# liulab-dfci/TRUST4

Measured on AMD Instinct MI355X. Metric: stage-1 assembly read pairs/sec (150 bp PE), whole stage 1, higher is better.
Workload: dtype int32/u64

## Files before the change

trust4_amd/csrc/t4_api.hip:

```cpp
#include <hip/hip_runtime.h>
#include <math.h>
#include <stdarg.h>
#include <stdio.h>
#include <string.h>
#include <zlib.h>

#include <algorithm>
#include <atomic>
#include <chrono>
#include <map>
#include <mutex>
#include <string>
#include <thread>
#include <unordered_map>
#include <vector>

#ifdef __HIPCC__
#include <dlfcn.h>
#include <rccl/rccl.h>
#include <type_traits>
#include <unistd.h>
#endif
#include "../../include/trust4_hip.h"
#include "t4_kernels.h"
// ... 230 lines not shown
  }
  int r;
  if (reads > w.maxReads) {
    int n = w.maxReads > 0 ? w.maxReads : 64;
    while (n < reads) n *= 2;
    if ((r = devAlloc(c, &w.seed, 2 * (size_t)n * T4_WIDE_SEEDS))) return r;
    if ((r = devAlloc(c, &w.bounds, 2 * (size_t)n * (T4_WIDE_MAXP + 1)))) return r;
    if ((r = devAlloc(c, &w.uniqPref, 2 * (size_t)n * (w.pcap + 1)))) return r;
    if ((r = devAlloc(c, &w.sortTmp, 2 * (size_t)n * 2 * w.pcap))) return r;
    w.maxReads = n;
  }
  if (parts > w.maxPart) {
    int n = w.maxPart > 0 ? w.maxPart : wideEnv("T4_WIDE_PARTS", 1024);
    while (n < parts) n *= 2;
    const size_t n2 = 2 * (size_t)n;
    if ((r = devAlloc(c, &w.pCnt, n2))) return r;
    if ((r = devAlloc(c, &w.pRead, n2))) return r;
    if ((r = devAlloc(c, &w.pKeys, n2 * w.pcap))) return r;
    if ((r = devAlloc(c, &w.gSize, n2 * w.pcap))) return r;
    if ((r = devAlloc(c, &w.gInfo, n2 * w.pcap))) return r;
    if ((r = devAlloc(c, &w.gCount, n2 * 4))) return r;
    if ((r = devAlloc(c, &w.gOff, n2 * 2))) return r;
    if ((r = devAlloc(c, &w.pRec, n2 * w.maxOvPart * 10))) return r;
    if ((r = devAlloc(c, &w.pRecCnt, n2))) return r;
    if ((r = devAlloc(c, &w.mKeys, n2 * w.maxOvPart))) return r;
    if ((r = devAlloc(c, &w.mOrd, n2 * w.maxOvPart))) return r;
    w.maxPart = n;
  }
  if (groups > w.grpCap) {
    int n = w.grpCap > 0 ? w.grpCap : wideEnv("T4_WIDE_GROUPS", 1 << 20);
    while (n < groups) n *= 2;
    if (c->grpPoolHost) (void)hipHostFree(c->grpPoolHost);
    c->grpPoolHost = nullptr; w.grpPool = nullptr;
    HIPCHK(c, hipHostMalloc(&c->grpPoolHost, sizeof(T4Grp) * 2 * (size_t)n, hipHostMallocMapped));
    HIPCHK(c, hipHostGetDevicePointer((void **)&w.grpPool, c->grpPoolHost, 0));
    w.grpCap = n;
  }
  return T4_OK;
}
T4Wide wideHalf(const t4_ctx *c, int half) {
  T4Wide w = c->wide;
  if (!half) return w;
  const size_t R = (size_t)w.maxReads, P = (size_t)w.maxPart;
  w.seed += R * T4_WIDE_SEEDS; w.bounds += R * (T4_WIDE_MAXP + 1); w.uniqPref += R * (w.pcap + 1); w.sortTmp += R * 2 * w.pcap;
  w.pCnt += P; w.pRead += P; w.pKeys += P * w.pcap; w.gSize += P * w.pcap; w.gInfo += P * w.pcap; w.gCount += P * 4; w.gOff += P * 2;
  w.pRec += P * w.maxOvPart * 10; w.pRecCnt += P; w.mKeys += P * w.maxOvPart; w.mOrd += P * w.maxOvPart;
  w.grpPool += w.grpCap;
  return w;
}

}

extern "C" {

int t4_init(int device_ordinal, t4_ctx **out) {
  if (!out) return T4_ERR_ARG;
  *out = nullptr;
  int ndev = 0;
  if (hipGetDeviceCount(&ndev) != hipSuccess || ndev <= 0 || device_ordinal < 0 || device_ordinal >= ndev) return T4_ERR_HIP;
  if (hipSetDevice(device_ordinal) != hipSuccess) return T4_ERR_HIP;
  t4_ctx *c = new t4_ctx();
  c->device = device_ordinal;
  hipDeviceProp_t prop;
  if (hipGetDeviceProperties(&prop, device_ordinal) != hipSuccess) { delete c; return T4_ERR_HIP; }
  c->cus = prop.multiProcessorCount;
  if (hipStreamCreate(&c->stream) != hipSuccess) { delete c; return T4_ERR_HIP; }
  for (int i = 0; i < 4; ++i) if (hipEventCreate(&c->ev[i]) != hipSuccess) { delete c; return T4_ERR_HIP; }
  memset(&c->stats, 0, sizeof c->stats);
  if (hipMalloc(&c->listCounts, sizeof(int) * 16) != hipSuccess || hipMalloc(&c->hitCounter, sizeof(unsigned long long)) != hipSuccess) { delete c; return T4_ERR_HIP; }
  if (hipHostMalloc(&c->aqFlagHost, 64, hipHostMallocMapped) != hipSuccess || hipHostGetDevicePointer((void **)&c->aqFlagDev, c->aqFlagHost, 0) != hipSuccess ||
      hipMalloc(&c->aqDoneCtr, sizeof(unsigned)) != hipSuccess || hipMemset(c->aqDoneCtr, 0, sizeof(unsigned)) != hipSuccess) { delete c; return T4_ERR_HIP; }
  *c->aqFlagHost = 0;
  *out = c;
  return T4_OK;
}

void t4_destroy(t4_ctx *c) {
  if (!c) return;
  (void)hipSetDevice(c->device);
#ifdef T4_PHASE_TIMING
  if (getenv("T4_PHASE_DUMP")) {
    unsigned long long ph[T4_NPHASE];
    if (hipMemcpyFromSymbol(ph, HIP_SYMBOL(t4k::g_phaseCycles), sizeof(ph)) == hipSuccess) {
      static const char *names[32] = {"other", "seed:lookup", "expand", "sort", "stats", "runs", "bigsort", "chain", "ovsort", "score", "prefilter", "final", "annotate", "score:quick", "score:banded", "score:finish", "extend:ungapped", "after-extend", "extend:list", "extend:dp4", "extend:dp1", "extend:combine", "seed:replay", "seed:scan", "extend:launch", "-", "-", "-", "-", "-", "-", "-"};
      unsigned long long tot = 0;
      for (int i = 0; i < T4_NPHASE; ++i) tot += ph[i];
      for (int i = 0; i < T4_NPHASE; ++i) if (ph[i]) fprintf(stderr, "phase %-16s %-7s %6.2f%%  %.3e cycles\n", names[i & 31], i < 32 ? "lds" : "global", 100.0 * (double)ph[i] / (double)tot, (double)ph[i]);
    }
    static unsigned long long cls[4 * T4_NPHASE];
    if (hipMemcpyFromSymbol(cls, HIP_SYMBOL(t4k::g_phaseByOverlaps), sizeof(cls)) == hipSuccess) {
      static const char *names[32] = {"other", "seed:lookup", "expand", "sort", "stats", "runs", "bigsort", "chain", "ovsort", "score", "prefilter", "final", "annotate", "score:quick", "score:banded", "score:finish", "extend:ungapped", "after-extend", "extend:list", "extend:dp4", "extend:dp1", "extend:combine", "seed:replay", "seed:scan", "extend:launch", "-", "-", "-", "-", "-", "-", "-"};
      static const char *cname[4] = {"<5 overlaps", "5-19 overlaps", "20-64 overlaps", ">64 overlaps"};
      for (int k = 0; k < 4; ++k) {
        unsigned long long tot = 0;
        for (int i = 0; i < T4_NPHASE; ++i) tot += cls[k * T4_NPHASE + i];
        if (!tot) continue;
        fprintf(stderr, "AddRead queries with %s: %.3e cycles in the query kernel\n", cname[k], (double)tot);
        for (int i = 0; i < T4_NPHASE; ++i) if (cls[k * T4_NPHASE + i] * 200 >= tot) fprintf(stderr, "   %-16s %-7s %6.2f%%\n", names[i & 31], i < 32 ? "lds" : "global", 100.0 * (double)cls[k * T4_NPHASE + i] / (double)tot);
      }
    }
    unsigned long long dc[8];
    if (hipMemcpyFromSymbol(dc, HIP_SYMBOL(t4k::g_dbgCount), sizeof(dc)) == hipSuccess)
      fprintf(stderr, "debug counters: gap jobs %llu, banded %llu, wave-DP steps %llu, scratch fallbacks %llu; overhang DPs %llu, of which %llu leave the diagonal\n", dc[0], dc[1], dc[2], dc[3], dc[6], dc[7]);
  }
#endif
  void *ptrs[] = {c->dpRows, c->dpDir, c->gKeys, c->gPairs, c->gCand, c->gOv, c->gFin, c->gOrd, c->hitsKeys, c->lists,
                  c->listCounts, c->status, c->counts, c->hitCounter, c->result, c->aqIn, c->aqOut};
  if (c->aqInHost) (void)hipHostFree(c->aqInHost);
  if (c->aqOutHost) (void)hipHostFree(c->aqOutHost);
  if (c->aqFlagHost) (void)hipHostFree(c->aqFlagHost);
  if (c->aqDoneCtr) (void)hipFree(c->aqDoneCtr);
  if (c->aqPool) (void)hipHostFree(c->aqPool);
  if (c->candPool) (void)hipHostFree(c->candPool);
  if (c->aqRecDev) (void)hipFree(c->aqRecDev);
  if (c->aqRecRead) (void)hipFree(c->aqRecRead);
  if (c->wideInit) {
    void *wp[] = {c->wide.seed, c->wide.bounds, c->wide.pCnt, c->wide.pRead, c->wide.pKeys, c->wide.gSize, c->wide.gInfo, c->wide.gCount, c->wide.gOff, c->wide.pRec,
                  c->wide.pRecCnt, c->wide.uniqPref, c->wide.mKeys, c->wide.mOrd, c->wide.sortTmp};
    for (void *p : wp) if (p) (void)hipFree(p);
    if (c->grpPoolHost) (void)hipHostFree(c->grpPoolHost);
  }
  for (void *p : ptrs) if (p) (void)hipFree(p);
  for (int i = 0; i < 4; ++i) if (c->ev[i]) (void)hipEventDestroy(c->ev[i]);
  if (c->stream) (void)hipStreamDestroy(c->stream);
  if (c->stream2) (void)hipStreamDestroy(c->stream2);
  if (c->evIn) (void)hipEventDestroy(c->evIn);
  if (c->evG) (void)hipEventDestroy(c->evG);
  delete c;
}

int t4_sync(t4_ctx *c) {
  if (!c) return T4_ERR_ARG;
  HIPCHK(c, hipStreamSynchronize(c->stream));
  return T4_OK;
}
const char *t4_last_error(t4_ctx *c) { return c ? c->err.c_str() : "null ctx"; }
int t4_device_cus(t4_ctx *c) { return c ? c->cus : 0; }
int t4_ctx_device(t4_ctx *c) { return c ? c->device : 0; }
#ifdef T4_PHASE_TIMING
int t4_debug_phase_cycles(unsigned long long *out16) {
  unsigned long long zero[T4_NPHASE] = {0};
  if (hipMemcpyFromSymbol(out16, HIP_SYMBOL(t4k::g_phaseCycles), sizeof(zero)) != hipSuccess) return T4_ERR_HIP;
  if (hipMemcpyToSymbol(HIP_SYMBOL(t4k::g_phaseCycles), zero, sizeof(zero)) != hipSuccess) return T4_ERR_HIP;
  return T4_OK;
}
int t4_debug_counters(unsigned long long *out8) {
  unsigned long long zero[8] = {0};
  if (hipMemcpyFromSymbol(out8, HIP_SYMBOL(t4k::g_dbgCount), sizeof(zero)) != hipSuccess) return T4_ERR_HIP;
  if (hipMemcpyToSymbol(HIP_SYMBOL(t4k::g_dbgCount), zero, sizeof(zero)) != hipSuccess) return T4_ERR_HIP;
  return T4_OK;
}
#endif
int t4_debug_phase_reset(void) {
#ifdef T4_PHASE_TIMING
  unsigned long long zero[T4_NPHASE] = {0};
  if (hipMemcpyToSymbol(HIP_SYMBOL(t4k::g_phaseCycles), zero, sizeof(zero)) != hipSuccess) return T4_ERR_HIP;
#endif
  return T4_OK;
}
int t4_last_stats(t4_ctx *c, t4_stats *out) {
  if (!c || !out) return T4_ERR_ARG;
  *out = c->stats;
  return T4_OK;
}

int t4_index_create(t4_ctx *c, int k, int consider_barcode, t4_index **out) {
  if (!c || !out) return T4_ERR_ARG;
  if (k < 2 || k > 31) return fail(c, T4_ERR_ARG, "kmer_length %d outside [2,31]", k);
  t4_index *ix = new t4_index();
  ix->ctx = c; ix->k = k; ix->considerBarcode = consider_barcode ? 1 : 0;
  double kmerHitProb = pow(0.8, k);
  ix->nomatchGapLimit = int(k * (log(0.01) / log(1 - kmerHitProb))) + 1;
  *out = ix;
  return T4_OK;
// ... 2339 lines not shown
```

trust4_amd/csrc/t4_kernels.h:

```cpp
#pragma once
#include <hip/hip_runtime.h>

#include "t4_device.h"

namespace t4k {

#ifdef T4_INLINE_ALL
#define T4_NI
#else
#define T4_NI __attribute__((noinline))
#endif
#ifndef T4_OPT_JOBSORT
#define T4_OPT_JOBSORT 1
#endif
#ifndef T4_OPT_ROWWALK
#define T4_OPT_ROWWALK 1
#endif
#ifndef T4_NI_R3
#define T4_NI_R3 0
#endif
#ifdef __HIPCC__
#define T4_LDS_AS __attribute__((address_space(3)))
#else
#define T4_LDS_AS
// ... 1471 lines not shown
  if (ix.radius > 0) {
    const int wave = lane >> 6, nw = NT >> 6, wl = lane & 63;
    for (int c = wave; c < nCand; c += nw) {
      int s = CAND_START(wm.cand[c]), n = CAND_LEN(wm.cand[c]);
      if (n <= 48) continue;
      unsigned long long ks = wm.keys[s];
      if (!seqIsRef(ix, KEY_IDX(ks))) continue;
      unsigned *tmp = (unsigned *)(wm.keys + s) + n;
      for (int t = wl; t < n; t += 64) {
        unsigned long long kt = wm.keys[s + t];
        int b = KEY_B(kt), a = KEY_C(kt) - T4_C_BIAS + b;
        wm.pairs[s + t] = ((unsigned)b << 12) | (unsigned)a;
      }
      waveLdsSync();
#if T4_OPT_R2CHECK
      {
        bool unsorted = false;
        for (int t = wl + 1; t < n; t += 64) unsorted = unsorted || wm.pairs[s + t - 1] > wm.pairs[s + t];
        if (!__any(unsorted)) continue;
      }
#endif
      for (int t = wl; t < n; t += 64) {
        unsigned v = wm.pairs[s + t];
        int rank = 0;
        for (int u = 0; u < n; ++u) { unsigned x = wm.pairs[s + u]; rank += (x < v) ? 1 : 0; }
        tmp[rank] = v;
      }
      waveLdsSync();
      for (int t = wl; t < n; t += 64) wm.pairs[s + t] = tmp[t];
      waveLdsSync();
    }
  }
  __syncthreads();
  PHASE_MARK(ws, 7);
#if T4_OPT_ROWCHAIN
  chainRunsRows(ix, wm, ws, nCand, hitLenRequired);
  __syncthreads();
}
#else
  for (int c = lane; c < nCand; c += NT) {
    int s = CAND_START(wm.cand[c]), n = CAND_LEN(wm.cand[c]);
    unsigned long long ks = wm.keys[s];
    int idx = KEY_IDX(ks), plus = KEY_PLUS(ks);
    bool isRef = seqIsRef(ix, idx);
    int adjustRadius = isRef ? ix.radius : 0;
    if (!(adjustRadius > 0 && n > 48)) {
      for (int t = s; t < s + n; ++t) {
        unsigned long long kt = wm.keys[t];
        int b = KEY_B(kt), a = KEY_C(kt) - T4_C_BIAS + b;
        wm.pairs[t] = ((unsigned)b << 12) | (unsigned)a;
      }
      if (adjustRadius > 0) {
        for (int t = s + 1; t < s + n; ++t) {
          unsigned v = wm.pairs[t];
          int u = t - 1;
          while (u >= s && wm.pairs[u] > v) { wm.pairs[u + 1] = wm.pairs[u]; --u; }
          wm.pairs[u + 1] = v;
        }
      }
    }
    chainRun(ix, wm, ws, s, n, idx, plus, isRef, hitLenRequired);
  }
  __syncthreads();
}
#endif

__device__ __forceinline__ bool lowComplex(const WaveMem &wm, bool plus, int rs, int re) {
  int lo = plus ? rs : wm.segLen - 1 - re, hi = plus ? re : wm.segLen - 1 - rs;
  lo += wm.segAbs; hi += wm.segAbs;
  int cA = 0, cC = 0, cG = 0, cT = 0;
  for (int w = lo >> 4; w <= (hi >> 4); ++w) {
    const unsigned x = wm.pkRow[w];
    unsigned nb = (wm.nmRow[w >> 1] >> ((w & 1) * 16)) & 0xFFFFu;
    nb = (nb | (nb << 8)) & 0x00FF00FFu; nb = (nb | (nb << 4)) & 0x0F0F0F0Fu;
    nb = (nb | (nb << 2)) & 0x33333333u; nb = (nb | (nb << 1)) & 0x55555555u;
    unsigned v = 0x55555555u & ~nb;
    const int b0 = w << 4;
    if (lo > b0) v &= ~0u << ((lo - b0) * 2);
    if (hi < b0 + 15) v &= ~0u >> ((b0 + 15 - hi) * 2);
    const unsigned l = x & 0x55555555u, h = (x >> 1) & 0x55555555u;
    cA += __popc(~h & ~l & v); cC += __popc(~h & l & v); cG += __popc(h & ~l & v); cT += __popc(h & l & v);
  }
  const int cnt[4] = {cA, cC, cG, cT};
  int lowCnt = 0, lowTotal = 0;
  for (int i = 0; i < 4; ++i) if (cnt[i] <= 2) { ++lowCnt; lowTotal += cnt[i]; }
  if (lowTotal * 7 >= re - rs + 1) return false;
  return lowCnt >= 2;
}

__device__ bool dpAffineQuick(const char *t, int lent, const char *p, int lenp, unsigned &cnt) {
  cnt = 0;
  if (lent == 0 || lenp == 0) return true;
  if (lent != lenp) return false;
  int mm = 0;
  for (int i = 0; i < lent; ++i) { char a = t[i], b = p[i]; mm += (a == b || a == 'N' || b == 'N') ? 0 : 1; }
  if (lent > 1 && mm > 3) return false;
  cnt = CNT_MATCH * (unsigned)(lent - mm) + CNT_MIS * (unsigned)mm;
  return true;
}
__device__ bool dpPosWeightQuick(const T4PW *w, int lent, const char *p, int lenp, unsigned &cnt) {
  cnt = 0;
  if (lent == 0 || lenp == 0) return true;
  if (lent != lenp) return false;
  int mm = 0;
  for (int i = 0; i < lent; ++i) mm += baseEqualW(w[i], p[i]) ? 0 : 1;
  if (lent > 1 && !((lent - mm) * 2 - mm * 2 >= lent * 2 - 8)) return false;
  cnt = CNT_MATCH * (unsigned)(lent - mm) + CNT_MIS * (unsigned)mm;
  return true;
}

template <bool PW>
__device__ unsigned dpWave(const char *t, const T4PW *w, int lent, const char *p, int lenp, char *tbuf) {
  const int d = laneId();
  if (lent == 0 || lenp == 0) return 0u;
  if (lent == 1 && lenp == 1) {
    bool eq = PW ? baseEqualW(w[0], p[0]) : (t[0] == p[0] || t[0] == 'N' || p[0] == 'N');
    return eq ? CNT_MATCH : CNT_MIS;
  }
  if (PW && lent == lenp) {
    int mm = 0;
    for (int i = d; i < lent; i += 64) mm += baseEqualW(w[i], p[i]) ? 0 : 1;
    mm = waveSum(mm);
    if ((lent - mm) * 2 - mm * 2 >= lent * 2 - 8) return CNT_MATCH * (unsigned)(lent - mm) + CNT_MIS * (unsigned)mm;
  }
  int leftBand = 5, rightBand = 5;
  if (lent > lenp) rightBand += lent - lenp; else if (lent < lenp) leftBand += lenp - lent;
  const int W = leftBand + rightBand + 1;
  if (W > 64 || lent > T4_MAXGAP || lenp > T4_MAXGAP) return DP_FAIL;
  for (int i = d; i < lent; i += 64) tbuf[i] = PW ? (char)w[i] : t[i];
  const int negInf = (lent + 1) * (lenp + 1) * (-4);
  const int e0 = -4 + (lenp + 1) * (-4);
  const int q4 = 4 * (lenp + 1);
  int M = negInf, E = negInf, F = negInf;
  unsigned C0 = 0, C1 = 0, C2 = 0;
  {
    int j0 = d - leftBand;
    if (d < W && j0 >= 0 && j0 <= lent) {
      if (j0 == 0) { M = 0; E = 0; F = 0; }
      else if (PW) { M = -4 - 4 * j0; C0 = CNT_MATCH + CNT_INDEL * (unsigned)(j0 - 1); }
      else { M = -4 - 4 * j0; E = e0; F = -4 - j0; C0 = CNT_INDEL * (unsigned)(j0 + (j0 > q4 ? 1 : 0)); C1 = CNT_INDEL * (unsigned)(1 + j0); C2 = CNT_INDEL * (unsigned)j0; }
    }
  }
  const int lastStep = 2 * lenp + W - 1;
  for (int s = 2; s <= lastStep; ++s) {
    int lM = waveUp1(M), uM = waveDown1(M);
    unsigned lC0 = waveUp1(C0), uC0 = waveDown1(C0);
    int lF = 0, uE = 0; unsigned lC2 = 0, uC1 = 0;
    if (!PW) { lF = waveUp1(F); lC2 = waveUp1(C2); uE = waveDown1(E); uC1 = waveDown1(C1); }
    const int i2 = s - d, i = i2 >> 1, j = i - leftBand + d;
    if (d < W && (i2 & 1) == 0 && i >= 1 && i <= lenp && j >= 1 && j <= lent) {
      if (j == 1) {
        lM = -4 - 4 * i;
        if (PW) lC0 = CNT_MATCH + CNT_INDEL * (unsigned)(i - 1);
        else { lF = -4 - 4 * i; lC0 = CNT_INDEL * (unsigned)i; lC2 = CNT_INDEL * (unsigned)(1 + i); }
      } else if (d == 0) { lM = negInf; lF = negInf; lC0 = 0; lC2 = 0; }
      if (i == 1) {
        uM = -4 - 4 * j;
        if (PW) uC0 = CNT_MATCH + CNT_INDEL * (unsigned)(j - 1);
        else { uE = e0; uC0 = CNT_INDEL * (unsigned)(j + (j > q4 ? 1 : 0)); uC1 = CNT_INDEL * (unsigned)(1 + j); }
      } else if (d + 1 >= W) { uM = negInf; uE = negInf; uC0 = 0; uC1 = 0; }
      int dM; unsigned dC0;
      if (i == 1) {
        int jj = j - 1;
        dM = jj == 0 ? 0 : -4 - 4 * jj;
        dC0 = jj == 0 ? 0u : (PW ? CNT_MATCH + CNT_INDEL * (unsigned)(jj - 1) : CNT_INDEL * (unsigned)(jj + (jj > q4 ? 1 : 0)));
      } else if (j == 1) {
// ... 278 lines not shown
  int anyFast = 0;
  if (ALL && !rowsForAll) {
    for (int i = lane; i < overlapCnt; i += NT) {
      OvRec oc = wm.ov[wm.ord[i]];
      if ((oc.flags & OV_ISREF) != 0 && ix.radius > 0) anyFast = 1;
      else walkOverlap(ix, wm, ws, oc, i, true);
    }
    if (blockSum(anyFast, ws->red) == 0) return;
  }
  for (int i0 = 0; i0 < overlapCnt; i0 += nRows) {
    const int i = i0 + row;
    const bool has = i < overlapCnt;
    int chainPos = 0, chainLen = 0, ovSlot = 0;
    bool fast = false;
    if (has) {
      ovSlot = wm.ord[i];
      const OvRec &o = wm.ov[ovSlot];
      chainPos = o.chainPos; chainLen = o.chainLen;
      fast = (o.flags & OV_ISREF) != 0 && ix.radius > 0;
      if (!ALL && !fast && rl == 0) { OvRec oc = o; walkOverlap(ix, wm, ws, oc, i, true); }
    }
    const unsigned *hc = (const unsigned *)(wm.keys + chainPos);
    int jStop = 0x7FFFFFFF;
    const bool slow = ALL && has && !fast && rowsForAll;
    if (slow)
      for (int j = 1 + rl; j < chainLen; j += 16) {
        const unsigned pp = hc[j - 1], cp = hc[j];
        const int pa = PA(pp), pb = PB(pp), qa = PA(cp), qb = PB(cp);
        if (pb - pa != qb - qa || (pa + K - 1 < qa && (qb - (pb + K) > ix.nomatchGapLimit || qa - (pa + K) > ix.nomatchGapLimit))) { jStop = j; break; }
      }
    if (fast)
      for (int j = 1 + rl; j < chainLen; j += 16) {
        const unsigned pp = hc[j - 1], cp = hc[j];
        const int pa = PA(pp), pb = PB(pp), qa = PA(cp), qb = PB(cp);
        const bool gapA = pa + K - 1 < qa, gapB = pb + K - 1 < qb;
        const bool doDP = (pb - pa == qb - qa) ? gapA : (gapA && gapB);
        if (doDP && (qb - (pb + K) > ix.nomatchGapLimit || qa - (pa + K) > ix.nomatchGapLimit)) { jStop = j; break; }
      }
    for (int m = 1; m < 16; m <<= 1) { const int other = __shfl_xor(jStop, m); jStop = other < jStop ? other : jStop; }
    int matchCnt = 0, indelCnt = 0;
    if (slow)
      for (int j = 1 + rl; j < chainLen && j < jStop; j += 16) {
        if (PA(hc[j - 1]) + K - 1 < PA(hc[j])) {
          const int slot = atomicAdd(&ws->jobCount, 1);
          if (slot < wm.candCap) wm.cand[slot] = (unsigned)i | ((unsigned)j << 16); else ws->overflow = 1;
        }
      }
    if (fast)
      for (int j = 1 + rl; j < chainLen && j <= jStop; j += 16) {
        if (j == jStop) { matchCnt += 2 * K; break; }
        const unsigned pp = hc[j - 1], cp = hc[j];
        const int pa = PA(pp), pb = PB(pp), qa = PA(cp), qb = PB(cp);
        bool doDP = false;
        if (pb - pa == qb - qa) {
          if (pa + K - 1 >= qa) matchCnt += 2 * (qa - pa);
          else { matchCnt += 2 * K; doDP = true; }
        } else if (pa + K - 1 >= qa && pb + K - 1 < qb) { matchCnt += 2 * (qa - pa); indelCnt += (qb - (pb + K) + (qa + K - pa)); }
        else if (pa + K - 1 < qa && pb + K - 1 >= qb) { matchCnt += 2 * (qb - pb); indelCnt += (qa - (pa + K) + (qb + K - pb)); }
        else if (pa + K - 1 >= qa && pb + K - 1 >= qb) {
          const int da = qa - pa, db = qb - pb;
          matchCnt += 2 * (da < db ? da : db);
          const int d = (qa - qb) - (pa - pb);
          indelCnt += d < 0 ? -d : d;
        } else { matchCnt += 2 * K; doDP = true; }
        if (doDP) {
          const int slot = atomicAdd(&ws->jobCount, 1);
          if (slot < wm.candCap) wm.cand[slot] = (unsigned)i | ((unsigned)j << 16); else ws->overflow = 1;
        }
      }
    matchCnt = rowSum16(matchCnt);
    indelCnt = rowSum16(indelCnt);
    if (fast && rl == 0) {
      ((unsigned *)hc)[chainLen] = (unsigned)(matchCnt + 2 * K);
      OvRec &dst = wm.ov[ovSlot];
      dst.indelCnt = indelCnt;
      if (jStop == 0x7FFFFFFF) dst.flags &= ~OV_SIMZERO; else dst.flags |= OV_SIMZERO;
    }
  }
}

__device__ T4_NI void finishOverlapsRows(const T4IndexView &ix, WaveMem &wm, WaveState *ws, int overlapCnt) {
  const int lane = tid(), NT = nthr(), K = ix.k;
  const int row = lane >> 4, rl = lane & 15, nRows = NT >> 4;
  for (int i0 = 0; i0 < overlapCnt; i0 += nRows) {
    const int i = i0 + row;
    const bool has = i < overlapCnt;
    OvRec o = wm.ov[wm.ord[has ? i : 0]];
    const bool fast = (o.flags & OV_ISREF) != 0 && ix.radius > 0;
    const int runSize = (o.flags & OV_ISREF) ? 0 : o.indelCnt;
    const unsigned *hc = (const unsigned *)(wm.keys + o.chainPos);
    const unsigned *res = hc + o.chainLen;
    int jBreak = 0x7FFFFFFF, add = 0, ind = 0, failed = 0;
    if (has && !fast)
      for (int j = 1 + rl; j < o.chainLen; j += 16) {
        const unsigned pp = hc[j - 1], cp = hc[j];
        const int pa = PA(pp), pb = PB(pp), qa = PA(cp), qb = PB(cp);
        bool stop = false;
        int a = 0;
        if (pb - pa != qb - qa) stop = true;
        else if (pa + K - 1 >= qa) a = 2 * (qa - pa);
        else {
          a = 2 * K;
          if (qb - (pb + K) > ix.nomatchGapLimit || qa - (pa + K) > ix.nomatchGapLimit) stop = true;
          else {
            const unsigned c = res[j];
            if (c == DP_FAIL) { stop = true; failed = 1; }
            else { a += 2 * (int)(c & 1023u); if (c >> 20) { stop = true; ind = (int)(c >> 20); } }
          }
        }
        if (stop) { jBreak = j; add += a; break; }
        add += a;
      }
    int jb = jBreak;
    for (int m = 1; m < 16; m <<= 1) { const int other = __shfl_xor(jb, m); jb = other < jb ? other : jb; }
    if (has && !fast && jb != 0x7FFFFFFF) {
      add = 0; 
      for (int j = 1 + rl; j < o.chainLen && j <= jb; j += 16) {
        const unsigned pp = hc[j - 1], cp = hc[j];
        const int pa = PA(pp), pb = PB(pp), qa = PA(cp), qb = PB(cp);
        if (pb - pa != qb - qa) continue;
        if (pa + K - 1 >= qa) { add += 2 * (qa - pa); continue; }
        add += 2 * K;
        if (qb - (pb + K) > ix.nomatchGapLimit || qa - (pa + K) > ix.nomatchGapLimit) continue;
        const unsigned c = res[j];
        if (c != DP_FAIL) add += 2 * (int)(c & 1023u);
      }
      if (jBreak != jb) { ind = 0; failed = 0; }
    }
    add = rowSum16(add);
    ind = rowSum16(ind);
    failed = rowSum16(failed);
    if (has && rl == 0) {
      const int m0 = o.matchCnt;
      if (fast) {
        o.matchCnt = (int)res[0];
        if (lowComplex(wm, (o.flags & OV_PLUS) != 0, o.rs, o.re)) o.flags |= OV_SIMZERO;
      } else {
        if (failed) ws->unsupported = 1;
        o.matchCnt = 2 * K + add; o.indelCnt = ind;
        if (jb == 0x7FFFFFFF) o.flags &= ~OV_SIMZERO; else o.flags |= OV_SIMZERO;
        if (lowComplex(wm, (o.flags & OV_PLUS) != 0, o.rs, o.re)) o.flags |= OV_SIMZERO;
      }
#ifdef T4_PATHDBG
      if (!fast) {
        OvRec chk = wm.ov[wm.ord[i]];
        walkOverlap(ix, wm, ws, chk, i, false);
        const int kind = jb == 0x7FFFFFFF ? 0 : failed ? 3 : ind ? 2 : 1;
        printf("PATHDBG finishrows kind %d %s\n", kind, (chk.matchCnt == o.matchCnt && chk.indelCnt == o.indelCnt && chk.flags == o.flags) ? "ok" : "MISMATCH");
      }
#endif
      o.chainLen = m0;
      if (!(o.flags & OV_ISREF)) ovKeepRunSize(o, runSize);
      wm.ov[wm.ord[i]] = o;
    }
  }
}
#endif

__device__ __forceinline__ void addGapResult(WaveMem &wm, WaveState *ws, int ovSlot, unsigned c) {
  OvRec &o = wm.ov[ovSlot];
  if (c == DP_FAIL) { ws->unsupported = 1; return; }
  unsigned *res0 = (unsigned *)(wm.keys + o.chainPos) + o.chainLen;
  atomicAdd(res0, 2u * (c & 1023u));
  if (c >> 20) atomicAdd(&o.indelCnt, (int)(c >> 20));
}

__device__ void runGapJobQuick(const T4IndexView &ix, WaveMem &wm, WaveState *ws, unsigned job) {
  const int K = ix.k;
  const OvRec &o = wm.ov[wm.ord[job & 0xFFFF]];
  const int j = (int)(job >> 16);
  unsigned *hc = (unsigned *)(wm.keys + o.chainPos);
  const int pa = PA(hc[j - 1]), pb = PB(hc[j - 1]), qa = PA(hc[j]), qb = PB(hc[j]);
  const int lent = qb - (pb + K), lenp = qa - (pa + K);
  const char *r = ((o.flags & OV_PLUS) ? wm.seg : wm.rc) + pa + K;
  const T4SeqInfo si = ix.seqs[o.seqIdx];
  unsigned cnt;
  bool done = si.isRef ? dpAffineQuick(ix.cons + si.consOff + pb + K, lent, r, lenp, cnt)
                       : dpPosWeightQuick(ix.pw + si.pwOff + pb + K, lent, r, lenp, cnt);
  hc[o.chainLen + j] = done ? cnt : DP_PENDING;
  if (done && si.isRef && ix.radius > 0) addGapResult(wm, ws, wm.ord[job & 0xFFFF], cnt);
}

__device__ int selectVJPair(const T4IndexView &ix, WaveMem &wm, int n) {
  int maxMatch = 0, tagi = 0, tagj = 0;
  for (int i = 0; i < n; ++i)
    for (int j = i + 1; j < n; ++j) {
      T4SeqInfo a = ix.seqs[wm.ov[i].seqIdx], b = ix.seqs[wm.ov[j].seqIdx];
      if (a.name0 != b.name0 || a.name1 != b.name1 || a.name2 != b.name2 || a.name3 == b.name3) continue;
      if (a.name3 == 'V') { if (wm.ov[i].rs > wm.ov[j].rs) continue; }
      else { if (wm.ov[i].rs < wm.ov[j].rs) continue; }
      if (wm.ov[i].matchCnt + wm.ov[j].matchCnt > maxMatch) { maxMatch = wm.ov[i].matchCnt + wm.ov[j].matchCnt; tagi = i; tagj = j; }
    }
  if (maxMatch == 0) return 0;
  OvRec a = wm.ov[tagi], b = wm.ov[tagj];
  wm.ov[0] = a; wm.ov[1] = b;
  return 2;
}

template <bool NOVEL>
__device__ int seedChainPass(const T4IndexView &ix, WaveMem &wm, WaveState *ws, int segLen, int strandArg, int barcode,
                             bool allowTotalSkip, bool vjOnly, int hitLenRequired, int filter, int onlySeq = -1) {
  const int lane = tid(), NT = nthr();
  unsigned *posStart = (unsigned *)wm.ov;
  unsigned *posPref = wm.pairs;
  const int nk = segLen - ix.k + 1;
  if (lane == 0) ws->ovCount = 0;
  PHASE_MARK(ws, 1);
  int H = NOVEL ? seedPositionsNovel(ix, wm, segLen, strandArg, barcode, allowTotalSkip, posStart, posPref, ws->red, wm.keys, ws)
                : seedPositions(ix, wm, segLen, strandArg, barcode, allowTotalSkip, posStart, posPref, ws->red);
  if (NOVEL && onlySeq >= 0) {
    __syncthreads();
    int Hv = expandHitsContig(ix, wm, ws, nk, onlySeq, posPref);
    const bool offContig = Hv != -2;
    if (!offContig) Hv = expandHitsOnly(ix, wm, ws, nk, H, onlySeq, posStart, posPref);
    if (Hv < 0) return -1;
    if (offContig) H = Hv;
    if (Hv > 1) { if (wm.ldsArrays) bitonicSortRegLds(wm.keys, Hv); else bitonicSort(wm.keys, Hv); }
    __syncthreads();
    int nPlus = 0;
    for (int i = lane; i < Hv; i += NT) nPlus += (int)(wm.keys[i] >> 63);
    nPlus = blockSum(nPlus, ws->red);
    if (lane == 0) { ws->hullLo[0] = ws->hullLo[1] = 0x7FFFFFFF; ws->hullHi[0] = ws->hullHi[1] = -0x7FFFFFFF; }
    __syncthreads();
    for (int i = lane; i < Hv; i += NT) {
      const unsigned long long ki = wm.keys[i];
      const unsigned long long dg = ki >> T4_B_BITS;
      if (i > 0 && (wm.keys[i - 1] >> T4_B_BITS) == dg) continue;
      if (i + 2 < Hv && (wm.keys[i + 2] >> T4_B_BITS) == dg) {
        const int at = -(KEY_C(ki) - T4_C_BIAS), st = KEY_PLUS(ki);
        atomicMin(&ws->hullLo[st], at);
        atomicMax(&ws->hullHi[st], at + segLen - 1);
      }
    }
    __syncthreads();
    overlapsFromKeys(ix, wm, ws, Hv, hitLenRequired, 0);
    if (lane == 0) {
      const int g[2] = {Hv - nPlus, nPlus};
// ... 581 lines not shown
  const int negInf = (L + 1) * (L + 1) * (-4);
  int M = negInf;
  unsigned S = PS_INDEL, fin = PS_INDEL;
  { int j0 = d - leftBand; if (d < W && j0 >= 0 && j0 <= L) M = j0 == 0 ? 0 : -4 - 4 * j0; }
  const int lastStep = 2 * L + W - 1;
  for (int s = 2; s <= lastStep; ++s) {
    int lM = waveUp1(M), uM = waveDown1(M);
    const unsigned lS = waveUp1(S), uS = waveDown1(S);
    const int i2 = s - d, i = i2 >> 1, j = i - leftBand + d;
    if (d < W && (i2 & 1) == 0 && i >= 1 && i <= L && j >= 1 && j <= L) {
      if (j == 1) lM = -4 - 4 * i; else if (d == 0) lM = negInf;
      if (i == 1) uM = -4 - 4 * j; else if (d + 1 >= W) uM = negInf;
      int dM;
      if (i == 1) dM = (j - 1 == 0) ? 0 : -4 - 4 * (j - 1);
      else if (j == 1) dM = -4 - 4 * (i - 1);
      else dM = M;
      const bool eq = baseEqualW(wst[j - 1], p[i - 1]);
      const int dsc = dM + (eq ? 2 : -2);
      int m = dsc;
      if (lM - 4 > m) m = lM - 4;
      if (uM - 4 > m) m = uM - 4;
      dirbuf[i * W + d] = (unsigned char)((lM - 4 == m ? 1 : 0) | (uM - 4 == m ? 2 : 0) | (dsc == m ? 4 : 0) | (eq ? 8 : 0));
      if (dsc == m) S = pathStepDiag((i == 1 && j == 1) ? 0u : ((i == 1 || j == 1) ? pathBorder(i + j - 2) : S), eq);
      else if (uM - 4 == m) S = (i == 1 ? pathBorder(j) : uS) | PS_INDEL;
      else S = (j == 1 ? pathBorder(i) : lS) | PS_INDEL;
      if (i == L && j == L) fin = S;
      M = m;
    }
  }
  return (unsigned)__shfl((int)fin, leftBand);
}
__device__ unsigned dpRowTracePW(const T4PW *w, int L, const char *p, unsigned char *dirbuf, int Lmax) {
  const int d = laneId() & 15, W = 11, leftBand = 5;
  unsigned char *wst = T4_EXT_WST(dirbuf, L);
  for (int t = d; t < L; t += 16) wst[t] = w[t];
  waveLdsSync();
  const int negInf = (L + 1) * (L + 1) * (-4);
  int M = negInf;
  unsigned S = PS_INDEL, fin = PS_INDEL;
  { int j0 = d - leftBand; if (d < W && j0 >= 0 && j0 <= L) M = j0 == 0 ? 0 : -4 - 4 * j0; }
  const int lastStep = 2 * Lmax + W - 1;
  for (int s = 2; s <= lastStep; ++s) {
    int lM = rowUp1(M), uM = rowDown1(M);
    const unsigned lS = rowUp1(S), uS = rowDown1(S);
    const int i2 = s - d, i = i2 >> 1, j = i - leftBand + d;
    if (d < W && (i2 & 1) == 0 && i >= 1 && i <= L && j >= 1 && j <= L) {
      if (j == 1) lM = -4 - 4 * i; else if (d == 0) lM = negInf;
      if (i == 1) uM = -4 - 4 * j; else if (d + 1 >= W) uM = negInf;
      int dM;
      if (i == 1) dM = (j - 1 == 0) ? 0 : -4 - 4 * (j - 1);
      else if (j == 1) dM = -4 - 4 * (i - 1);
      else dM = M;
      const bool eq = baseEqualW(wst[j - 1], p[i - 1]);
      const int dsc = dM + (eq ? 2 : -2);
      int m = dsc;
      if (lM - 4 > m) m = lM - 4;
      if (uM - 4 > m) m = uM - 4;
      dirbuf[i * W + d] = (unsigned char)((lM - 4 == m ? 1 : 0) | (uM - 4 == m ? 2 : 0) | (dsc == m ? 4 : 0) | (eq ? 8 : 0));
      if (dsc == m) S = pathStepDiag((i == 1 && j == 1) ? 0u : ((i == 1 || j == 1) ? pathBorder(i + j - 2) : S), eq);
      else if (uM - 4 == m) S = (i == 1 ? pathBorder(j) : uS) | PS_INDEL;
      else S = (j == 1 ? pathBorder(i) : lS) | PS_INDEL;
      if (i == L && j == L) fin = S;
      M = m;
    }
  }
  return (unsigned)__shfl((int)fin, (laneId() & ~15) + leftBand);
}
__device__ void dpRowPairLean(const unsigned char *wstA, int LA, const char *pA, const unsigned char *wstB, int LB, const char *pB,
                              int Lmax, unsigned long long &outA, unsigned long long &outB) {
  const int d = laneId() & 15, W = 11, leftBand = 5;
  typedef const T4_LDS_AS unsigned char *LdsB;
  typedef const T4_LDS_AS char *LdsC;
  const bool odd = (d & 1) != 0;
  const int LE = odd ? LB : LA, LO = odd ? LA : LB;
  const LdsB wE = (LdsB)(odd ? wstB : wstA), wO = (LdsB)(odd ? wstA : wstB);
  const LdsC pE = (LdsC)(odd ? pB : pA), pO = (LdsC)(odd ? pA : pB);
  const int negE = (LE + 1) * (LE + 1) * (-4), negO = (LO + 1) * (LO + 1) * (-4);
  const bool inBand = d < W, first = d == 0, last = d + 1 >= W;
  int ME = 0, MO = 0, RE = 0, RO = 0;
  unsigned SE = PS_INDEL, SO = PS_INDEL;
  int iE = (2 - d - (odd ? 1 : 0)) >> 1;
  int iO = (3 - d - (odd ? 0 : 1)) >> 1;
  const int nPair = (2 * Lmax + W) / 2 + 1;
#define T4_PAIR_STEP(Mself, Mnb, Sself, Snb, Rself, L_, w_, p_, neg_, i_)                                                               \
  {                                                                                                                                   \
    int lM = rowUp1(Mnb), uM = rowDown1(Mnb);                                                                                          \
    const unsigned lS = rowUp1(Snb), uS = rowDown1(Snb);                                                                               \
    const int i = (i_), j = i - leftBand + d;                                                                                          \
    if (inBand && (unsigned)(i - 1) < (unsigned)(L_) && (unsigned)(j - 1) < (unsigned)(L_)) {                                          \
      if (j == 1) lM = -4 - 4 * i; else if (first) lM = (neg_);                                                                        \
      if (i == 1) uM = -4 - 4 * j; else if (last) uM = (neg_);                                                                         \
      const int dM = i == 1 ? (j == 1 ? 0 : -4 * j) : (j == 1 ? -4 * i : Mself);                                                       \
      const bool eq = baseEqualW((w_)[j - 1], (p_)[i - 1]);                                                                            \
      const int dsc = dM + (eq ? 2 : -2);                                                                                              \
      int m = dsc;                                                                                                                     \
      if (lM - 4 > m) m = lM - 4;                                                                                                      \
      if (uM - 4 > m) m = uM - 4;                                                                                                      \
      if (dsc == m) { Sself = pathStepDiag((i == 1 && j == 1) ? 0u : ((i == 1 || j == 1) ? pathBorder(i + j - 2) : Sself), eq); Rself = (i == 1 ? 0 : Rself) + 1; } \
      else if (uM - 4 == m) { Sself = (i == 1 ? pathBorder(j) : uS) | PS_INDEL; Rself = 0; }                                           \
      else { Sself = (j == 1 ? pathBorder(i) : lS) | PS_INDEL; Rself = 0; }                                                            \
      Mself = m;                                                                                                                       \
    }                                                                                                                                  \
  }
  for (int u = 0; u < nPair; ++u) {
    T4_PAIR_STEP(ME, MO, SE, SO, RE, LE, wE, pE, negE, iE)
    T4_PAIR_STEP(MO, ME, SO, SE, RO, LO, wO, pO, negO, iO)
    ++iE; ++iO;
  }
#undef T4_PAIR_STEP
  const int src = (laneId() & ~15) + leftBand;
  const unsigned sA = (unsigned)__shfl((int)SO, src), sB = (unsigned)__shfl((int)SE, src);
  const unsigned rA = (unsigned)__shfl(RO, src), rB = (unsigned)__shfl(RE, src);
  outA = (unsigned long long)sA | ((unsigned long long)rA << 32);
  outB = (unsigned long long)sB | ((unsigned long long)rB << 32);
}
__device__ int tracebackPW(const unsigned char *dirbuf, int L, signed char *align) {
  const int W = 11, leftBand = 5;
  int tagi = L, tagj = L, tag = 0;
  while (tagi > 0 || tagj > 0) {
    int a = 0;
    if (tagi > 0 && tagj > 0) {
      unsigned char bits = dirbuf[tagi * W + (tagj - tagi + leftBand)];
      if (bits & 1) a = 3;
      if (bits & 2) a = 2;
      if (bits & 4) a = (bits & 8) ? 0 : 1;
    } else if (tagi == 0) {
      int mL = (tagj - 1 == 0) ? 0 : (-4 - 4 * (tagj - 1));
      if (mL - 4 == -4 - 4 * tagj) a = 3;
    } else {
      int mU = (tagi - 1 == 0) ? 0 : (-4 - 4 * (tagi - 1));
      if (mU - 4 == -4 - 4 * tagi) a = 2;
    }
    align[tag++] = (signed char)a;
    if (a == 3) --tagj; else if (a == 2) --tagi; else { --tagi; --tagj; }
  }
  for (int i = 0, j = tag - 1; i < j; ++i, --j) { signed char x = align[i]; align[i] = align[j]; align[j] = x; }
  return tag;
}

__device__ void extendOverlaps(const T4IndexView &ix, WaveMem &wm, WaveState *ws, int n, int len, bool useFirstStrand,
                               double factor, ExtSide *sides, unsigned char *dirbuf, int dirBytes, ExtOut *res, bool lean = false) {
  const int lane = tid(), NT = nthr();
  const int plus0 = n > 0 ? (wm.fin[wm.ord[0]].flags & OV_PLUS) : 1;
  {
    const int wave = lane >> 6, nwv = NT >> 6, wl = lane & 63;
    for (int q = wave; q < 2 * n; q += nwv) {
      const OvRec &o = wm.fin[wm.ord[q >> 1]];
      const int side = q & 1;
      const T4SeqInfo si = ix.seqs[o.seqIdx];
      const char *r = (useFirstStrand ? plus0 : (o.flags & OV_PLUS)) ? wm.seg : wm.rc;
      int size, t0, p0;
      if (side == 0) { size = o.rs < o.ss ? o.rs : o.ss; t0 = o.ss - size; p0 = o.rs - size; }
      else { int a = len - 1 - o.re, b = si.len - 1 - o.se; size = a < b ? a : b; t0 = o.se + 1; p0 = o.re + 1; }
      const T4PW *w = ix.pw + si.pwOff + t0;
      int mm = 0, good = 0, tmpBase = 0;
      for (int base = 0; base < size; base += 64) {
        const int k = base + wl;
        const int pos = side == 0 ? size - 1 - k : k;
        const bool in = k < size;
        const bool eq = in && baseEqualW(w[pos], r[p0 + pos]);
        const unsigned long long bal = __ballot(eq);
        const int tmp = tmpBase + __popcll(bal & ((wl == 63) ? ~0ull : ((2ull << wl) - 1ull)));
        const unsigned long long gb = __ballot(eq && tmp > 0.75 * (k + 1));
        if (gb) good = base + 64 - __clzll((long long)gb);
        mm += __popcll(__ballot(in && !eq));
        tmpBase += __popcll(bal);
      }
      if (wl == 0) {
        ExtSide e;
        e.size = (short)size; e.match = (short)(size - mm); e.mis = (short)mm; e.indel = 0; e.pending = 0;
        if (size > 1 && !((size - mm) * 2 - mm * 2 >= size * 2 - 8)) e.pending = 1;
        e.good = (short)good;
        sides[q] = e;
      }
    }
  }
  __syncthreads();
  PHASE_MARK(ws, 18);
  if (lean) {
    int nPend = 0, maxL = 0;
    for (int q0 = 0; q0 < 2 * n; q0 += NT) {
      const int q = q0 + lane;
      const bool pend = q < 2 * n && sides[q].pending;
      int tot;
      const int inc = blockInclScan(pend ? 1 : 0, ws->red, tot);
      if (pend) wm.cand[nPend + inc - 1] = (unsigned)q;
      nPend += tot;
      int mx;
      blockInclMaxScan(pend ? (int)sides[q].size : 0, ws->red, mx);
      if (mx > maxL) maxL = mx;
// ... 1322 lines not shown
```

Measured before the change: 17540.

## Parallelize chain rewalk and low-complexity check across row lanes, prefetch DP base compares

The chain walk in finishOverlapsRows now steps in 16-wide lockstep chunks. It uses a ballot to find the first stopping link, which replaces the per-lane break followed by a second re-walk pass. The low-complexity base counting is spread over the 16 lanes of a row with packed counters and a row reduction, instead of running serially on lane 0. In the paired banded DP, base-equality loads are prefetched one step ahead with clamped indices to take LDS latency off the dependency chain. The changes add ballot and shuffle traffic and extra clamped loads, and the chunked walk may run more iterations for rows with short chains.

Result: slower. 17300 (-1.3%).

```diff
diff --git a/trust4_amd/csrc/t4_api.hip b/trust4_amd/csrc/t4_api.hip
--- a/trust4_amd/csrc/t4_api.hip
+++ b/trust4_amd/csrc/t4_api.hip
@@ -336,14 +336,14 @@
   if (getenv("T4_PHASE_DUMP")) {
     unsigned long long ph[T4_NPHASE];
     if (hipMemcpyFromSymbol(ph, HIP_SYMBOL(t4k::g_phaseCycles), sizeof(ph)) == hipSuccess) {
-      static const char *names[32] = {"other", "seed:lookup", "expand", "sort", "stats", "runs", "bigsort", "chain", "ovsort", "score", "prefilter", "final", "annotate", "score:quick", "score:banded", "score:finish", "extend:ungapped", "after-extend", "extend:list", "extend:dp4", "extend:dp1", "extend:combine", "seed:replay", "seed:scan", "extend:launch", "-", "-", "-", "-", "-", "-", "-"};
+      static const char *names[32] = {"other", "seed:lookup", "expand", "sort", "stats", "runs", "bigsort", "chain", "ovsort", "score", "prefilter", "final", "annotate", "score:quick", "score:banded", "score:finish", "extend:ungapped", "after-extend", "extend:list", "extend:dp4", "extend:dp1", "extend:combine", "seed:replay", "seed:scan", "extend:launch", "score:rewalk", "score:tail", "-", "-", "-", "-", "-"};
       unsigned long long tot = 0;
       for (int i = 0; i < T4_NPHASE; ++i) tot += ph[i];
       for (int i = 0; i < T4_NPHASE; ++i) if (ph[i]) fprintf(stderr, "phase %-16s %-7s %6.2f%%  %.3e cycles\n", names[i & 31], i < 32 ? "lds" : "global", 100.0 * (double)ph[i] / (double)tot, (double)ph[i]);
     }
     static unsigned long long cls[4 * T4_NPHASE];
     if (hipMemcpyFromSymbol(cls, HIP_SYMBOL(t4k::g_phaseByOverlaps), sizeof(cls)) == hipSuccess) {
-      static const char *names[32] = {"other", "seed:lookup", "expand", "sort", "stats", "runs", "bigsort", "chain", "ovsort", "score", "prefilter", "final", "annotate", "score:quick", "score:banded", "score:finish", "extend:ungapped", "after-extend", "extend:list", "extend:dp4", "extend:dp1", "extend:combine", "seed:replay", "seed:scan", "extend:launch", "-", "-", "-", "-", "-", "-", "-"};
+      static const char *names[32] = {"other", "seed:lookup", "expand", "sort", "stats", "runs", "bigsort", "chain", "ovsort", "score", "prefilter", "final", "annotate", "score:quick", "score:banded", "score:finish", "extend:ungapped", "after-extend", "extend:list", "extend:dp4", "extend:dp1", "extend:combine", "seed:replay", "seed:scan", "extend:launch", "score:rewalk", "score:tail", "-", "-", "-", "-", "-"};
       static const char *cname[4] = {"<5 overlaps", "5-19 overlaps", "20-64 overlaps", ">64 overlaps"};
       for (int k = 0; k < 4; ++k) {
         unsigned long long tot = 0;
diff --git a/trust4_amd/csrc/t4_kernels.h b/trust4_amd/csrc/t4_kernels.h
--- a/trust4_amd/csrc/t4_kernels.h
+++ b/trust4_amd/csrc/t4_kernels.h
@@ -1577,6 +1577,31 @@
     cA += __popc(~h & ~l & v); cC += __popc(~h & l & v); cG += __popc(h & ~l & v); cT += __popc(h & l & v);
   }
   const int cnt[4] = {cA, cC, cG, cT};
+  int lowCnt = 0, lowTotal = 0;
+  for (int i = 0; i < 4; ++i) if (cnt[i] <= 2) { ++lowCnt; lowTotal += cnt[i]; }
+  if (lowTotal * 7 >= re - rs + 1) return false;
+  return lowCnt >= 2;
+}
+
+__device__ __forceinline__ bool lowComplexRow(const WaveMem &wm, bool plus, int rs, int re, int rl) {
+  int lo = plus ? rs : wm.segLen - 1 - re, hi = plus ? re : wm.segLen - 1 - rs;
+  lo += wm.segAbs; hi += wm.segAbs;
+  int cAC = 0, cGT = 0;
+  for (int w = (lo >> 4) + rl; w <= (hi >> 4); w += 16) {
+    const unsigned x = wm.pkRow[w];
+    unsigned nb = (wm.nmRow[w >> 1] >> ((w & 1) * 16)) & 0xFFFFu;
+    nb = (nb | (nb << 8)) & 0x00FF00FFu; nb = (nb | (nb << 4)) & 0x0F0F0F0Fu;
+    nb = (nb | (nb << 2)) & 0x33333333u; nb = (nb | (nb << 1)) & 0x55555555u;
+    unsigned v = 0x55555555u & ~nb;
+    const int b0 = w << 4;
+    if (lo > b0) v &= ~0u << ((lo - b0) * 2);
+    if (hi < b0 + 15) v &= ~0u >> ((b0 + 15 - hi) * 2);
+    const unsigned l = x & 0x55555555u, h = (x >> 1) & 0x55555555u;
+    cAC += __popc(~h & ~l & v) | (__popc(~h & l & v) << 16);
+    cGT += __popc(h & ~l & v) | (__popc(h & l & v) << 16);
+  }
+  cAC = rowSum16(cAC); cGT = rowSum16(cGT);
+  const int cnt[4] = {cAC & 0xFFFF, (int)((unsigned)cAC >> 16), cGT & 0xFFFF, (int)((unsigned)cGT >> 16)};
   int lowCnt = 0, lowTotal = 0;
   for (int i = 0; i < 4; ++i) if (cnt[i] <= 2) { ++lowCnt; lowTotal += cnt[i]; }
   if (lowTotal * 7 >= re - rs + 1) return false;
@@ -2021,6 +2046,7 @@
 __device__ T4_NI void finishOverlapsRows(const T4IndexView &ix, WaveMem &wm, WaveState *ws, int overlapCnt) {
   const int lane = tid(), NT = nthr(), K = ix.k;
   const int row = lane >> 4, rl = lane & 15, nRows = NT >> 4;
+  const int rowShift = laneId() & 48;
   for (int i0 = 0; i0 < overlapCnt; i0 += nRows) {
     const int i = i0 + row;
     const bool has = i < overlapCnt;
@@ -2029,13 +2055,17 @@
     const int runSize = (o.flags & OV_ISREF) ? 0 : o.indelCnt;
     const unsigned *hc = (const unsigned *)(wm.keys + o.chainPos);
     const unsigned *res = hc + o.chainLen;
-    int jBreak = 0x7FFFFFFF, add = 0, ind = 0, failed = 0;
-    if (has && !fast)
-      for (int j = 1 + rl; j < o.chainLen; j += 16) {
+    const int nWalk = (has && !fast) ? o.chainLen : 0;
+    int nMax = nWalk;
+    { int x = __shfl_xor(nMax, 16); if (x > nMax) nMax = x; x = __shfl_xor(nMax, 32); if (x > nMax) nMax = x; }
+    int jb = 0x7FFFFFFF, add = 0, ind = 0, failed = 0;
+    for (int j0 = 1; j0 < nMax; j0 += 16) {
+      const int j = j0 + rl;
+      bool stop = false;
+      int a = 0, aInd = 0, aFail = 0;
+      if (j < nWalk && jb == 0x7FFFFFFF) {
         const unsigned pp = hc[j - 1], cp = hc[j];
         const int pa = PA(pp), pb = PB(pp), qa = PA(cp), qb = PB(cp);
-        bool stop = false;
-        int a = 0;
         if (pb - pa != qb - qa) stop = true;
         else if (pa + K - 1 >= qa) a = 2 * (qa - pa);
         else {
@@ -2043,42 +2073,36 @@
           if (qb - (pb + K) > ix.nomatchGapLimit || qa - (pa + K) > ix.nomatchGapLimit) stop = true;
           else {
             const unsigned c = res[j];
-            if (c == DP_FAIL) { stop = true; failed = 1; }
-            else { a += 2 * (int)(c & 1023u); if (c >> 20) { stop = true; ind = (int)(c >> 20); } }
+            if (c == DP_FAIL) { stop = true; aFail = 1; }
+            else { a += 2 * (int)(c & 1023u); if (c >> 20) { stop = true; aInd = (int)(c >> 20); } }
           }
         }
-        if (stop) { jBreak = j; add += a; break; }
-        add += a;
-      }
-    int jb = jBreak;
-    for (int m = 1; m < 16; m <<= 1) { const int other = __shfl_xor(jb, m); jb = other < jb ? other : jb; }
-    if (has && !fast && jb != 0x7FFFFFFF) {
-      add = 0; 
-      for (int j = 1 + rl; j < o.chainLen && j <= jb; j += 16) {
-        const unsigned pp = hc[j - 1], cp = hc[j];
-        const int pa = PA(pp), pb = PB(pp), qa = PA(cp), qb = PB(cp);
-        if (pb - pa != qb - qa) continue;
-        if (pa + K - 1 >= qa) { add += 2 * (qa - pa); continue; }
-        add += 2 * K;
-        if (qb - (pb + K) > ix.nomatchGapLimit || qa - (pa + K) > ix.nomatchGapLimit) continue;
-        const unsigned c = res[j];
-        if (c != DP_FAIL) add += 2 * (int)(c & 1023u);
-      }
-      if (jBreak != jb) { ind = 0; failed = 0; }
-    }
+      }
+      const unsigned stops = (unsigned)(__ballot(stop) >> rowShift) & 0xFFFFu;
+      if (stops) {
+        const int first = __ffsll((unsigned long long)stops) - 1;
+        jb = j0 + first;
+        if (rl > first) a = 0;
+        if (rl != first) { aInd = 0; aFail = 0; }
+      }
+      add += a; ind += aInd; failed += aFail;
+      if (!__any(j0 + 16 < nWalk && jb == 0x7FFFFFFF)) break;
+    }
+    PHASE_MARK(ws, 26);
     add = rowSum16(add);
     ind = rowSum16(ind);
     failed = rowSum16(failed);
+    const bool lowC = lowComplexRow(wm, (o.flags & OV_PLUS) != 0, o.rs, o.re, rl);
     if (has && rl == 0) {
       const int m0 = o.matchCnt;
       if (fast) {
         o.matchCnt = (int)res[0];
-        if (lowComplex(wm, (o.flags & OV_PLUS) != 0, o.rs, o.re)) o.flags |= OV_SIMZERO;
+        if (lowC) o.flags |= OV_SIMZERO;
       } else {
         if (failed) ws->unsupported = 1;
         o.matchCnt = 2 * K + add; o.indelCnt = ind;
         if (jb == 0x7FFFFFFF) o.flags &= ~OV_SIMZERO; else o.flags |= OV_SIMZERO;
-        if (lowComplex(wm, (o.flags & OV_PLUS) != 0, o.rs, o.re)) o.flags |= OV_SIMZERO;
+        if (lowC) o.flags |= OV_SIMZERO;
       }
 #ifdef T4_PATHDBG
       if (!fast) {
@@ -2092,6 +2116,7 @@
       if (!(o.flags & OV_ISREF)) ovKeepRunSize(o, runSize);
       wm.ov[wm.ord[i]] = o;
     }
+    PHASE_MARK(ws, 15);
   }
 }
 #endif
@@ -2839,7 +2864,14 @@
   int iE = (2 - d - (odd ? 1 : 0)) >> 1;
   int iO = (3 - d - (odd ? 0 : 1)) >> 1;
   const int nPair = (2 * Lmax + W) / 2 + 1;
-#define T4_PAIR_STEP(Mself, Mnb, Sself, Snb, Rself, L_, w_, p_, neg_, i_)                                                               \
+  const int hiE = LE > 0 ? LE - 1 : 0, hiO = LO > 0 ? LO - 1 : 0;
+  auto eqAt = [&](LdsB w_, LdsC p_, int hi_, int i_) -> bool {
+    int ii = i_ - 1, jj = i_ - 1 - leftBand + d;
+    ii = ii < 0 ? 0 : (ii > hi_ ? hi_ : ii);
+    jj = jj < 0 ? 0 : (jj > hi_ ? hi_ : jj);
+    return baseEqualW(w_[jj], p_[ii]);
+  };
+#define T4_PAIR_STEP(Mself, Mnb, Sself, Snb, Rself, L_, eq_, neg_, i_)                                                                  \
   {                                                                                                                                   \
     int lM = rowUp1(Mnb), uM = rowDown1(Mnb);                                                                                          \
     const unsigned lS = rowUp1(Snb), uS = rowDown1(Snb);                                                                               \
@@ -2848,7 +2880,7 @@
       if (j == 1) lM = -4 - 4 * i; else if (first) lM = (neg_);                                                                        \
       if (i == 1) uM = -4 - 4 * j; else if (last) uM = (neg_);                                                                         \
       const int dM = i == 1 ? (j == 1 ? 0 : -4 * j) : (j == 1 ? -4 * i : Mself);                                                       \
-      const bool eq = baseEqualW((w_)[j - 1], (p_)[i - 1]);                                                                            \
+      const bool eq = (eq_);                                                                                                           \
       const int dsc = dM + (eq ? 2 : -2);                                                                                              \
       int m = dsc;                                                                                                                     \
       if (lM - 4 > m) m = lM - 4;                                                                                                      \
@@ -2859,10 +2891,12 @@
       Mself = m;                                                                                                                       \
     }                                                                                                                                  \
   }
+  bool eqE = eqAt(wE, pE, hiE, iE), eqO = eqAt(wO, pO, hiO, iO);
   for (int u = 0; u < nPair; ++u) {
-    T4_PAIR_STEP(ME, MO, SE, SO, RE, LE, wE, pE, negE, iE)
-    T4_PAIR_STEP(MO, ME, SO, SE, RO, LO, wO, pO, negO, iO)
-    ++iE; ++iO;
+    const bool nextE = eqAt(wE, pE, hiE, iE + 1), nextO = eqAt(wO, pO, hiO, iO + 1);
+    T4_PAIR_STEP(ME, MO, SE, SO, RE, LE, eqE, negE, iE)
+    T4_PAIR_STEP(MO, ME, SO, SE, RO, LO, eqO, negO, iO)
+    ++iE; ++iO; eqE = nextE; eqO = nextO;
   }
 #undef T4_PAIR_STEP
   const int src = (laneId() & ~15) + leftBand;
```
